# OllieBoyne/FIND

Hardware: AMD Instinct MI355X
Metric: deformed vertices x rendered views / sec (fwd+bwd) (higher is better)
Workload: dtype f32; 1 GPU; train_3d.yaml network-stage step: 16 feet x 6890-vertex template per GPU, 10002-vertex GT scans, chamf(5000)+smooth+texture(1000) losses, backward, Adam(main_params) step; nothing rendered, views:=1; feet_per_gpu=16, template_verts=6890, parallelism=dp1

## Files before the change

find_amd/csrc/geom.hip:

```cpp
#include "common.h"

namespace find {
namespace geom {

__device__ __forceinline__ float3 ld3(const float* p) { return make_float3(p[0], p[1], p[2]); }
__device__ __forceinline__ float3 sub3(float3 a, float3 b) { return make_float3(a.x - b.x, a.y - b.y, a.z - b.z); }
__device__ __forceinline__ float3 cross3(float3 a, float3 b) {
	return make_float3(a.y * b.z - a.z * b.y, a.z * b.x - a.x * b.z, a.x * b.y - a.y * b.x);
}
__device__ __forceinline__ float norm3(float3 a) { return sqrtf(a.x * a.x + a.y * a.y + a.z * a.z); }

__global__ void face_areas_kernel(const float* __restrict__ verts, const int32_t* __restrict__ faces, int64_t faces_mesh_stride,
								  int n_verts, int n_faces, float* __restrict__ areas) {
	const int m = blockIdx.y;
	const int f = blockIdx.x * blockDim.x + threadIdx.x;
	if (f >= n_faces) return;
	const int32_t* fp = faces + (int64_t)m * faces_mesh_stride + (int64_t)f * 3;
	const float* vp = verts + (int64_t)m * n_verts * 3;
	if (fp[0] < 0) {
		areas[(int64_t)m * n_faces + f] = 0.f;
		return;
	}
	const float3 a = ld3(vp + 3 * fp[0]), b = ld3(vp + 3 * fp[1]), c = ld3(vp + 3 * fp[2]);
	areas[(int64_t)m * n_faces + f] = 0.5f * norm3(cross3(sub3(b, a), sub3(c, a)));
// ... 419 lines not shown
					if (nn_dist(fx, fy, fz, s[0], s[1], s[2]) == best[k]) jj = j;
				}
			}
			key[k] = nn_key(best[k], jj);
		}
	}
	if (wave) {
#pragma unroll
		for (int k = 0; k < NQ; ++k) pkey[wave - 1][k * 64 + lane] = key[k];
	}
	__syncthreads();
	if (wave == 0) {
		float* dist = dir ? a.d[1].dist : a.d[0].dist;
		int32_t* idx = dir ? a.d[1].idx : a.d[0].idx;
		unsigned long long* kout = dir ? a.d[1].key : a.d[0].key;
#pragma unroll
		for (int k = 0; k < NQ; ++k) {
			unsigned long long b = key[k];
#pragma unroll
			for (int w = 0; w < 3; ++w) b = min(b, pkey[w][k * 64 + lane]);
			if (qi[k] >= p1_max) continue;
			const int64_t o = (int64_t)n * p1_max + qi[k];
			const bool valid = qi[k] < p1 && b != ~0ull;
			if (kout) {
				if (a.splits == 1) kout[o] = qi[k] < p1 ? b : ~0ull;
				else if (valid) atomicMin(kout + o, b);
			}
			if (dist) dist[o] = valid ? __uint_as_float((unsigned)(b >> 32)) : 0.f;
			if (idx) idx[o] = valid ? (int)(unsigned)b : -1;
		}
	}
}

__global__ __launch_bounds__(1024) void chamfer_reduce_kernel(const unsigned long long* __restrict__ kx, const int32_t* __restrict__ x_len, int p1_max,
															  const unsigned long long* __restrict__ ky, const int32_t* __restrict__ y_len, int p2_max,
															  int n_clouds, float* __restrict__ partial, unsigned* __restrict__ counter,
															  float* __restrict__ loss) {
	__shared__ float red[16];
	__shared__ bool last;
	const int n = blockIdx.x, dir = blockIdx.y;
	const unsigned long long* k = dir ? ky : kx;
	const int32_t* len = dir ? y_len : x_len;
	const int pmax = dir ? p2_max : p1_max;
	const int p = len ? len[n] : pmax;
	float s = 0.f;
	for (int i = threadIdx.x; i < p; i += 1024) {
		const unsigned long long v = k[(int64_t)n * pmax + i];
		s += v == ~0ull ? 0.f : __uint_as_float((unsigned)(v >> 32));
	}
	s = wave_sum(s);
	if ((threadIdx.x & 63) == 0) red[threadIdx.x >> 6] = s;
	__syncthreads();
	if (threadIdx.x == 0) {
		float t = 0.f;
		for (int w = 0; w < 16; ++w) t += red[w];
		partial[dir * n_clouds + n] = t / (float)max(p, 1);
		__threadfence();
		last = atomicAdd(counter, 1u) == 2u * n_clouds - 1u;
	}
	__syncthreads();
	if (last && threadIdx.x == 0) {
		__threadfence();
		float total = 0.f;
		for (int i = 0; i < 2 * n_clouds; ++i) total += __builtin_nontemporal_load(partial + i);
		*loss = total / (float)max(n_clouds, 1);
	}
// ... 212 lines not shown
__global__ __launch_bounds__(256) void chamfer_surface_sum_kernel(const float* __restrict__ slabs, int n_slices, int64_t slab_stride, int V3,
																  float* __restrict__ d_verts) {
	const int n = blockIdx.y, e = blockIdx.x * 256 + threadIdx.x;
	if (e >= V3) return;
	const float* p = slabs + (int64_t)n * n_slices * slab_stride + e;
	float s = 0.f;
	for (int k = 0; k < n_slices; ++k) s += p[(int64_t)k * slab_stride];
	d_verts[(int64_t)n * V3 + e] = s;
}

__global__ void nn_bwd_kernel(const float* __restrict__ x, const int32_t* __restrict__ x_len, const float* __restrict__ y,
							  const int32_t* __restrict__ idx, const float* __restrict__ w, int p1_max, int p2_max,
							  float* __restrict__ d_x, float* __restrict__ d_y) {
	const int n = blockIdx.y;
	const int i = blockIdx.x * blockDim.x + threadIdx.x;
	const int p1 = x_len ? x_len[n] : p1_max;
	if (i >= p1) return;
	const int64_t o = (int64_t)n * p1_max + i;
	const int j = idx[o];
	if (j < 0) return;
	const float g = 2.0f * w[o];
	const float* xp = x + o * 3;
	const float* yp = y + ((int64_t)n * p2_max + j) * 3;
	const float gx = g * (xp[0] - yp[0]), gy = g * (xp[1] - yp[1]), gz = g * (xp[2] - yp[2]);
	if (d_x) {
		d_x[o * 3 + 0] += gx; d_x[o * 3 + 1] += gy; d_x[o * 3 + 2] += gz;
	}
	if (d_y) {
		float* dy = d_y + ((int64_t)n * p2_max + j) * 3;
		atomicAdd(dy + 0, -gx); atomicAdd(dy + 1, -gy); atomicAdd(dy + 2, -gz);
	}
}

__global__ void cot_weights_kernel(const float* __restrict__ verts, const int32_t* __restrict__ faces, int n_verts, int n_faces,
								   float* __restrict__ fw) {
#pragma clang fp contract(off)
	const int m = blockIdx.y;
	const int f = blockIdx.x * blockDim.x + threadIdx.x;
	if (f >= n_faces) return;
	const int32_t* fp = faces + (int64_t)f * 3;
	const float* vp = verts + (int64_t)m * n_verts * 3;
	const float3 v0 = ld3(vp + 3 * fp[0]), v1 = ld3(vp + 3 * fp[1]), v2 = ld3(vp + 3 * fp[2]);
	const float A = norm3(sub3(v1, v2)), B = norm3(sub3(v0, v2)), C = norm3(sub3(v0, v1));
	const float s = 0.5f * (A + B + C);
	const float area = sqrtf(fmaxf(s * (s - A) * (s - B) * (s - C), 1e-12f));
	const float A2 = A * A, B2 = B * B, C2 = C * C;
	float* o = fw + ((int64_t)m * n_faces + f) * 3;
	o[0] = (B2 + C2 - A2) / area / 4.0f;
	o[1] = (A2 + C2 - B2) / area / 4.0f;
	o[2] = (A2 + B2 - C2) / area / 4.0f;
}

__device__ __forceinline__ float quad_sum(float v) {
	v += __shfl_xor(v, 1, 64);
	v += __shfl_xor(v, 2, 64);
	return v;
}

template <typename Q>
__device__ __forceinline__ void apply_L(Q qv, const int32_t* __restrict__ faces, const float* __restrict__ fw,
										const int32_t* __restrict__ vf_off, const int32_t* __restrict__ vf_items, int i, int t, bool live,
										float3* r, float* rowsum) {
	float3 acc = make_float3(0.f, 0.f, 0.f);
	float rs = 0.f;
	if (live) {
		const int hi = vf_off[i + 1];
		for (int e = vf_off[i] + t; e < hi; e += 4) {
			const int item = vf_items[e];
			const int f = item / 3, c = item - f * 3;
			const int c1 = (c + 1) % 3, c2 = (c + 2) % 3;
			const int j1 = faces[f * 3 + c1], j2 = faces[f * 3 + c2];
			const float w1 = fw[f * 3 + c2], w2 = fw[f * 3 + c1];
			const float3 a = qv(j1), b = qv(j2);
			acc.x += w1 * a.x + w2 * b.x; acc.y += w1 * a.y + w2 * b.y; acc.z += w1 * a.z + w2 * b.z;
			rs += w1 + w2;
		}
	}
	*r = make_float3(quad_sum(acc.x), quad_sum(acc.y), quad_sum(acc.z));
	*rowsum = quad_sum(rs);
}

constexpr int SMOOTH_VPB = 64;

__global__ __launch_bounds__(256) void smooth_fwd_kernel(const float* __restrict__ verts, const int32_t* __restrict__ faces,
														   const float* __restrict__ fw, const int32_t* __restrict__ vf_off,
														   const int32_t* __restrict__ vf_items, const int32_t* __restrict__ nbr_off,
														   const int32_t* __restrict__ nbr_idx, int n_verts, int n_faces,
														   float* __restrict__ nw_out, float* __restrict__ lapdir_out,
														   float* __restrict__ partial ) {
	const int m = blockIdx.y;
	const int i = blockIdx.x * SMOOTH_VPB + ((int)threadIdx.x >> 2), t = threadIdx.x & 3;
	const bool live = i < n_verts;
	const float* vp = verts + (int64_t)m * n_verts * 3;
	float3 r;
	float rs;
	apply_L([&](int j) { return ld3(vp + 3 * j); }, faces, fw + (int64_t)m * n_faces * 3, vf_off, vf_items, i, t, live, &r, &rs);
	float lap_n = 0.f, edge_s = 0.f;
	if (live) {
		const float3 v = ld3(vp + 3 * i);
		const int hi = nbr_off[i + 1];
		for (int e = nbr_off[i] + t; e < hi; e += 4) {
			const float3 d = sub3(v, ld3(vp + 3 * nbr_idx[e]));
			edge_s += d.x * d.x + d.y * d.y + d.z * d.z;
		}
		if (t == 0) {
			const float nw = rs > 0.f ? 1.0f / rs : rs;
			const float3 lap = make_float3(r.x * nw - v.x, r.y * nw - v.y, r.z * nw - v.z);
			lap_n = norm3(lap);
			const float inv = lap_n > 0.f ? 1.0f / lap_n : 0.f;
			const int64_t o = (int64_t)m * n_verts + i;
			nw_out[o] = nw;
			lapdir_out[o * 3 + 0] = lap.x * inv; lapdir_out[o * 3 + 1] = lap.y * inv; lapdir_out[o * 3 + 2] = lap.z * inv;
		}
	}
	__shared__ float red[2][4];
	const float a = wave_sum(lap_n), b = wave_sum(edge_s);
	if ((threadIdx.x & 63) == 0) { red[0][threadIdx.x >> 6] = a; red[1][threadIdx.x >> 6] = b; }
	__syncthreads();
	if (threadIdx.x < 2) {
		float sum = 0.f;
		for (int w = 0; w < 4; ++w) sum += red[threadIdx.x][w];
		partial[((int64_t)m * gridDim.x + blockIdx.x) * 2 + threadIdx.x] = sum;
	}
}

__global__ void smooth_finalize_kernel(const float* __restrict__ partial, int n_meshes, int nblk, int n_verts, int n_edges,
									   float* __restrict__ loss_edge, float* __restrict__ loss_lap, float w_edge, float w_lap,
									   float* __restrict__ loss_sum) {
	float lap = 0.f, edge = 0.f;
	for (int k = threadIdx.x; k < n_meshes * nblk; k += 64) { lap += partial[k * 2 + 0]; edge += partial[k * 2 + 1]; }
	lap = wave_sum(lap);
	edge = wave_sum(edge);
	if (threadIdx.x == 0) {
		const float l = lap / (float)n_verts / (float)n_meshes, e = 0.5f * edge / (float)n_edges / (float)n_meshes;
		if (loss_lap) *loss_lap = l;
		if (loss_edge) *loss_edge = e;
		if (loss_sum) *loss_sum = w_lap * l + w_edge * e;
	}
}

__global__ __launch_bounds__(256) void smooth_bwd_kernel(const float* __restrict__ verts, const int32_t* __restrict__ faces,
														   const float* __restrict__ fw, const int32_t* __restrict__ vf_off,
														   const int32_t* __restrict__ vf_items, const int32_t* __restrict__ nbr_off,
														   const int32_t* __restrict__ nbr_idx, const float* __restrict__ nw,
														   const float* __restrict__ lapdir, const float* __restrict__ g_edge,
														   const float* __restrict__ g_lap, float s_edge, float s_lap, int n_meshes, int n_verts,
														   int n_faces, int n_edges, float* __restrict__ d_verts) {
	const int m = blockIdx.y;
	const int i = blockIdx.x * SMOOTH_VPB + ((int)threadIdx.x >> 2), t = threadIdx.x & 3;
	const bool live = i < n_verts;
	const float* vp = verts + (int64_t)m * n_verts * 3;
	const float* nwp = nw + (int64_t)m * n_verts;
	const float* ldp = lapdir + (int64_t)m * n_verts * 3;
	const float su = (*g_lap) * s_lap / (float)n_verts / (float)n_meshes;
	float3 r;
	float rs;
	apply_L([&](int j) { const float sj = su * nwp[j]; const float3 u = ld3(ldp + 3 * j); return make_float3(sj * u.x, sj * u.y, sj * u.z); },
			faces, fw + (int64_t)m * n_faces * 3, vf_off, vf_items, i, t, live, &r, &rs);
	float3 es = make_float3(0.f, 0.f, 0.f);
	float3 v = es;
	if (live) {
		v = ld3(vp + 3 * i);
		const int hi = nbr_off[i + 1];
		for (int e = nbr_off[i] + t; e < hi; e += 4) {
			const float3 d = sub3(v, ld3(vp + 3 * nbr_idx[e]));
			es.x += d.x; es.y += d.y; es.z += d.z;
		}
	}
	es = make_float3(quad_sum(es.x), quad_sum(es.y), quad_sum(es.z));
	if (live && t == 0) {
		const int64_t o = (int64_t)m * n_verts + i;
		const float se = 2.0f * (*g_edge) * s_edge / (float)n_edges / (float)n_meshes;
		d_verts[o * 3 + 0] = r.x - su * ldp[3 * i + 0] + se * es.x;
		d_verts[o * 3 + 1] = r.y - su * ldp[3 * i + 1] + se * es.y;
		d_verts[o * 3 + 2] = r.z - su * ldp[3 * i + 2] + se * es.z;
	}
}

struct SmoothWs {
	float* fw;
	float* nw;
	float* lapdir;
	float* partial;
	int nblk;
	int64_t bytes;
};

static void carve_smooth(int64_t n_meshes, int64_t n_verts, int64_t n_faces, void* ws, SmoothWs* o) {
	Carver c(ws);
	o->nblk = (int)cdiv(n_verts, SMOOTH_VPB);
	o->fw = c.take<float>(n_meshes * n_faces * 3);
	o->nw = c.take<float>(n_meshes * n_verts);
	o->lapdir = c.take<float>(n_meshes * n_verts * 3);
	o->partial = c.take<float>(n_meshes * o->nblk * 2);
	o->bytes = c.off;
}

}
}

using namespace find;
using namespace find::geom;

static inline bool bad_dims(int64_t a, int64_t b) { return a < 1 || b < 1 || a >= (1 << 16) || b >= (1ll << 30); }

extern "C" int find_face_areas(const float* verts, const int32_t* faces, int64_t faces_batch, int64_t n_meshes, int64_t n_verts,
							   int64_t n_faces, float* areas, void* stream) {
	FIND_REQUIRE(verts && faces && areas, "find_face_areas: NULL argument");
	FIND_REQUIRE(!bad_dims(n_meshes, n_faces) && n_verts >= 1, "find_face_areas: bad sizes");
	FIND_REQUIRE(faces_batch == 1 || faces_batch == n_meshes, "find_face_areas: faces_batch must be 1 or n_meshes");
	hipLaunchKernelGGL(face_areas_kernel, dim3((unsigned)cdiv(n_faces, 256), (unsigned)n_meshes), dim3(256), 0, (hipStream_t)stream, verts,
					   faces, faces_batch == 1 ? 0 : n_faces * 3, (int)n_verts, (int)n_faces, areas);
	FIND_LAUNCH_CHECK("face_areas_kernel");
	return FIND_OK;
}

extern "C" int find_sample_points_fwd(const float* verts, const int32_t* faces, int64_t faces_batch, const int32_t* face_idx,
									  const float* uv, int64_t n_meshes, int64_t n_verts, int64_t n_faces, int64_t n_samples,
									  float* out, const float* attr, float* attr_out, void* stream) {
	FIND_REQUIRE(verts && faces && face_idx && uv && out, "find_sample_points_fwd: NULL argument");
	FIND_REQUIRE((attr == nullptr) == (attr_out == nullptr), "find_sample_points_fwd: attr and attr_out must both be given or both NULL");
	FIND_REQUIRE(!bad_dims(n_meshes, n_samples) && n_verts >= 1 && n_faces >= 1, "find_sample_points_fwd: bad sizes");
	FIND_REQUIRE(faces_batch == 1 || faces_batch == n_meshes, "find_sample_points_fwd: faces_batch must be 1 or n_meshes");
	hipLaunchKernelGGL(sample_fwd_kernel, dim3((unsigned)cdiv(n_samples, 256), (unsigned)n_meshes), dim3(256), 0, (hipStream_t)stream, verts,
					   faces, faces_batch == 1 ? 0 : n_faces * 3, face_idx, uv, (int)n_verts, (int)n_samples, out, attr, attr_out);
	FIND_LAUNCH_CHECK("sample_fwd_kernel");
	return FIND_OK;
// ... 146 lines not shown
				const bool face = (z == cz - r) || (z == cz + r) || (yy == cy - r) || (yy == cy + r);
				if (face || r == 0) scan_row(z, yy, x0, x1);
				else {
					if (cx - r >= 0) scan_row(z, yy, cx - r, cx - r);
					if (cx + r <= NG - 1) scan_row(z, yy, cx + r, cx + r);
				}
			}
		if (x0 == 0 && x1 == NG - 1 && y0 == 0 && y1 == NG - 1 && z0 == 0 && z1 == NG - 1) break;
		float gap = INFINITY;
		const float mx = 1e-4f * clx + 6e-7f * fmaxf(fabsf(ox), fabsf(qx)), my = 1e-4f * cly + 6e-7f * fmaxf(fabsf(oy), fabsf(qy)),
					mz = 1e-4f * clz + 6e-7f * fmaxf(fabsf(oz), fabsf(qz));
		if (cx - r > 0) gap = fminf(gap, rx - (cx - r) * clx - mx);
		if (cx + r < NG - 1) gap = fminf(gap, (cx + r + 1) * clx - rx - mx);
		if (cy - r > 0) gap = fminf(gap, ry - (cy - r) * cly - my);
		if (cy + r < NG - 1) gap = fminf(gap, (cy + r + 1) * cly - ry - my);
		if (cz - r > 0) gap = fminf(gap, rz - (cz - r) * clz - mz);
		if (cz + r < NG - 1) gap = fminf(gap, (cz + r + 1) * clz - rz - mz);
		gap = fmaxf(gap, 0.f);
		if (best != ~0ull && __uint_as_float((unsigned)(best >> 32)) < gap * gap * 0.9999f) break;
	}
	kout[qi] = best;
}

constexpr int TILE_PTS = 64;
constexpr int TILE_MAX_TILES = 128;
constexpr int TILE_MAX_POINTS = TILE_PTS * TILE_MAX_TILES;
struct TileDir {
	const float* p;
	const int32_t* len;
	int p_max;
	float4* sorted;
	float4* tab;
};
struct TileBuildArgs { TileDir d[2]; };

__device__ __forceinline__ unsigned tile_ord(float f) {
	const unsigned b = __float_as_uint(f);
	return b ^ ((b >> 31) ? 0xffffffffu : 0x80000000u);
}
__device__ __forceinline__ float tile_unord(unsigned u) { return __uint_as_float(u ^ ((u >> 31) ? 0x80000000u : 0xffffffffu)); }
__device__ __forceinline__ int tile_bin(float v, float lo, float scale) { return (int)fminf(fmaxf((v - lo) * scale, 0.f), 63.f); }

__device__ __forceinline__ unsigned tile_wave_max(unsigned v) {
	v = max(v, (unsigned)__builtin_amdgcn_update_dpp(0, (int)v, 0xB1, 0xf, 0xf, true));
	v = max(v, (unsigned)__builtin_amdgcn_update_dpp(0, (int)v, 0x4E, 0xf, 0xf, true));
	v = max(v, (unsigned)__builtin_amdgcn_update_dpp(0, (int)v, 0x141, 0xf, 0xf, true));
	v = max(v, (unsigned)__builtin_amdgcn_update_dpp(0, (int)v, 0x140, 0xf, 0xf, true));
	return max(max((unsigned)__builtin_amdgcn_readlane((int)v, 0), (unsigned)__builtin_amdgcn_readlane((int)v, 16)),
			   max((unsigned)__builtin_amdgcn_readlane((int)v, 32), (unsigned)__builtin_amdgcn_readlane((int)v, 48)));
}

__device__ __forceinline__ int tile_wave_scan(int v, int lane) {
	v += __builtin_amdgcn_update_dpp(0, v, 0x111, 0xf, 0xf, true);
	v += __builtin_amdgcn_update_dpp(0, v, 0x112, 0xf, 0xf, true);
	v += __builtin_amdgcn_update_dpp(0, v, 0x114, 0xf, 0xf, true);
	v += __builtin_amdgcn_update_dpp(0, v, 0x118, 0xf, 0xf, true);
	const int r0 = __builtin_amdgcn_readlane(v, 15), r1 = __builtin_amdgcn_readlane(v, 31), r2 = __builtin_amdgcn_readlane(v, 47);
	return v + (lane >= 16 ? r0 : 0) + (lane >= 32 ? r1 : 0) + (lane >= 48 ? r2 : 0);
}
__device__ __forceinline__ int tile_widest(float ex, float ey, float ez) {
	return (ey > ex && ey >= ez) ? 1 : (ez > ex && ez > ey) ? 2 : 0;
}

__global__ __launch_bounds__(1024) void nn_tile_build_kernel(const TileBuildArgs a) {
	constexpr int PPT = TILE_MAX_POINTS / 1024, MT = TILE_MAX_TILES;
	__shared__ int hist[MT / 2 * 64];
	__shared__ int n_m[2][MT];
	__shared__ int n_cnt[MT], n_start[MT], n_axis[MT];
	__shared__ float n_lo[3][MT], n_hi[3][MT];
	__shared__ float4 n_par[MT];
	__shared__ int4 s_split[MT];
	__shared__ int s_taken[MT];
	__shared__ unsigned b_lo[3][MT], b_hi[3][MT];
	__shared__ unsigned red[6][16];
	const int dir = blockIdx.y, n = blockIdx.x;
	const float* __restrict__ pts = dir ? a.d[1].p : a.d[0].p;
	const int32_t* len = dir ? a.d[1].len : a.d[0].len;
	const int p_max = dir ? a.d[1].p_max : a.d[0].p_max;
	const int p = min(max(len ? len[n] : p_max, 0), p_max);
	const int M = (p + TILE_PTS - 1) / TILE_PTS;
	if (M == 0 || M > MT) return;
	float4* sorted = (dir ? a.d[1].sorted : a.d[0].sorted) + (int64_t)n * p_max;
	float4* tab = (dir ? a.d[1].tab : a.d[0].tab) + (int64_t)n * ((p_max + TILE_PTS - 1) / TILE_PTS) * 2;
	const float* pp = pts + (int64_t)n * p_max * 3;
	const int tid = threadIdx.x, lane = tid & 63, wave = tid >> 6;
	const int kmax = (p + 1023) >> 10;
	float px[PPT], py[PPT], pz[PPT];
	int node[PPT], bin[PPT];
	bool own[PPT];
	float lo[3] = {INFINITY, INFINITY, INFINITY}, hi[3] = {-INFINITY, -INFINITY, -INFINITY};
#pragma unroll
	for (int k = 0; k < PPT; ++k) {
		const int j = k * 1024 + tid;
		own[k] = j < p;
		node[k] = 0;
		bin[k] = 0;
		const int jj = min(j, p - 1);
		px[k] = pp[(int64_t)jj * 3]; py[k] = pp[(int64_t)jj * 3 + 1]; pz[k] = pp[(int64_t)jj * 3 + 2];
		lo[0] = fminf(lo[0], px[k]); hi[0] = fmaxf(hi[0], px[k]);
		lo[1] = fminf(lo[1], py[k]); hi[1] = fmaxf(hi[1], py[k]);
		lo[2] = fminf(lo[2], pz[k]); hi[2] = fmaxf(hi[2], pz[k]);
	}
#pragma unroll
	for (int c = 0; c < 3; ++c) {
		const unsigned l = tile_wave_max(~tile_ord(lo[c])), h = tile_wave_max(tile_ord(hi[c]));
		if (lane == 0) { red[c][wave] = l; red[3 + c][wave] = h; }
	}
	for (int i = tid; i < MT / 2 * 64; i += 1024) hist[i] = 0;
	if (tid < MT) {
		n_m[0][tid] = 0; n_m[1][tid] = 0; s_taken[tid] = 0;
		s_split[tid] = make_int4(0, 0, 0, 0);
#pragma unroll
		for (int c = 0; c < 3; ++c) { b_lo[c][tid] = 0xffffffffu; b_hi[c][tid] = 0u; }
// ... 97 lines not shown
	__syncthreads();
	int pos[PPT];
#pragma unroll
	for (int k = 0; k < PPT; ++k) pos[k] = own[k] ? n_start[node[k]] + atomicAdd(&s_taken[node[k]], 1) : -1;
#pragma unroll
	for (int k = 0; k < PPT; ++k) {
		if (!own[k]) continue;
		const int f = node[k];
		atomicMin(&b_lo[0][f], tile_ord(px[k])); atomicMax(&b_hi[0][f], tile_ord(px[k]));
		atomicMin(&b_lo[1][f], tile_ord(py[k])); atomicMax(&b_hi[1][f], tile_ord(py[k]));
		atomicMin(&b_lo[2][f], tile_ord(pz[k])); atomicMax(&b_hi[2][f], tile_ord(pz[k]));
	}
#pragma unroll
	for (int k = 0; k < PPT; ++k)
		if (pos[k] >= 0 && pos[k] < p) sorted[pos[k]] = make_float4(px[k], py[k], pz[k], __int_as_float(k * 1024 + tid));
	__syncthreads();
	if (tid < M) {
		tab[2 * tid] = make_float4(tile_unord(b_lo[0][tid]), tile_unord(b_lo[1][tid]), tile_unord(b_lo[2][tid]), __int_as_float(n_start[tid]));
		tab[2 * tid + 1] = make_float4(tile_unord(b_hi[0][tid]), tile_unord(b_hi[1][tid]), tile_unord(b_hi[2][tid]), __int_as_float(n_cnt[tid]));
	}
}

struct TileQueryDir {
	const float4* qsorted;
	const float4* qtab;
	const int32_t* q_len;
	int q_max;
	const float4* tsorted;
	const float4* ttab;
	const int32_t* t_len;
	int t_max;
	unsigned long long* key;
};
struct TileQueryArgs { TileQueryDir d[2]; unsigned* counter; };

__global__ __launch_bounds__(256) void nn_tile_query_kernel(const TileQueryArgs a) {
	__shared__ float4 tl[4][TILE_PTS / 8 * 6];
	__shared__ int ti[4][TILE_PTS];
	const int dir = blockIdx.z, n = blockIdx.y;
	if (a.counter && (blockIdx.x | blockIdx.y | blockIdx.z | threadIdx.x) == 0) *a.counter = 0u;
	const int q_max = dir ? a.d[1].q_max : a.d[0].q_max, t_max = dir ? a.d[1].t_max : a.d[0].t_max;
	const int32_t* q_len = dir ? a.d[1].q_len : a.d[0].q_len;
	const int32_t* t_len = dir ? a.d[1].t_len : a.d[0].t_len;
	const int p1 = min(max(q_len ? q_len[n] : q_max, 0), q_max), p2 = min(max(t_len ? t_len[n] : t_max, 0), t_max);
	unsigned long long* kout = (dir ? a.d[1].key : a.d[0].key) + (int64_t)n * q_max;
	for (int r = p1 + blockIdx.x * 256 + threadIdx.x; r < q_max; r += gridDim.x * 256) kout[r] = ~0ull;
	const int lane = threadIdx.x & 63, wave = threadIdx.x >> 6;
	const int qt = __builtin_amdgcn_readfirstlane(blockIdx.x * 4 + wave);
	if (qt >= (p1 + TILE_PTS - 1) / TILE_PTS) return;
	const float4* __restrict__ qsorted = (dir ? a.d[1].qsorted : a.d[0].qsorted) + (int64_t)n * q_max;
	const float4* __restrict__ qtab = (dir ? a.d[1].qtab : a.d[0].qtab) + (int64_t)n * ((q_max + TILE_PTS - 1) / TILE_PTS) * 2;
	const float4* __restrict__ tsorted = (dir ? a.d[1].tsorted : a.d[0].tsorted) + (int64_t)n * t_max;
	const float4* __restrict__ ttab = (dir ? a.d[1].ttab : a.d[0].ttab) + (int64_t)n * ((t_max + TILE_PTS - 1) / TILE_PTS) * 2;
	const float4 qb0 = qtab[2 * qt], qb1 = qtab[2 * qt + 1];
	const int qstart = __builtin_amdgcn_readfirstlane(__float_as_int(qb0.w)), qcnt = __builtin_amdgcn_readfirstlane(__float_as_int(qb1.w));
	if (qcnt <= 0) return;
	const float4 q = qsorted[min(max(qstart, 0) + min(lane, qcnt - 1), p1 - 1)];
	const int ntt = (p2 + TILE_PTS - 1) / TILE_PTS;
	float lb[2];
	int tstart[2], tcnt[2];
#pragma unroll
	for (int h = 0; h < 2; ++h) {
		const int t = h * 64 + lane;
		lb[h] = INFINITY; tstart[h] = 0; tcnt[h] = 0;
		if (t < ntt) {
			const float4 b0 = ttab[2 * t], b1 = ttab[2 * t + 1];
			const float gx = fmaxf(0.f, fmaxf(b0.x - qb1.x, qb0.x - b1.x)), gy = fmaxf(0.f, fmaxf(b0.y - qb1.y, qb0.y - b1.y)),
						gz = fmaxf(0.f, fmaxf(b0.z - qb1.z, qb0.z - b1.z));
			lb[h] = __builtin_fmaf(gz, gz, __builtin_fmaf(gy, gy, gx * gx));
			tstart[h] = __float_as_int(b0.w); tcnt[h] = __float_as_int(b1.w);
		}
	}
	unsigned ord[2] = {lane < ntt ? __float_as_uint(lb[0]) : ~0u, 64 + lane < ntt ? __float_as_uint(lb[1]) : ~0u};
	unsigned picked_lb = ~0u;
	auto pick = [&]() -> int {
		picked_lb = ~tile_wave_max(~min(ord[0], ord[1]));
		if (picked_lb == ~0u) return -1;
		const unsigned long long b0 = __ballot(ord[0] == picked_lb);
		const int tt = b0 ? __builtin_ctzll(b0) : 64 + __builtin_ctzll(__ballot(ord[1] == picked_lb));
		if (lane == (tt & 63)) { if (tt < 64) ord[0] = ~0u; else ord[1] = ~0u; }
		return tt;
	};
	const v2f qx = {q.x, q.x}, qy = {q.y, q.y}, qz = {q.z, q.z};
	float best = INFINITY;
	int gj = 0;
	unsigned long long tie = ~0ull;
	float4* L = tl[wave];
	int* LI = ti[wave];
	float4 v = make_float4(0.f, 0.f, 0.f, 0.f);
// ... 29 lines not shown
			const int gn = min(g + 1, ng - 1);
#pragma unroll
			for (int i = 0; i < 6; ++i) B[i] = L[6 * gn + i];
#define FIND_TILE_D2(X, Y, Z, lo, hi) ({ const v2f dx = qx - v2f{X.lo, X.hi}, dy = qy - v2f{Y.lo, Y.hi}, dz = qz - v2f{Z.lo, Z.hi};   \
										 __builtin_elementwise_fma(dz, dz, __builtin_elementwise_fma(dy, dy, dx * dx)); })
			const v2f d0 = FIND_TILE_D2(A[0], A[2], A[4], x, y), d1 = FIND_TILE_D2(A[0], A[2], A[4], z, w);
			const v2f d2 = FIND_TILE_D2(A[1], A[3], A[5], x, y), d3 = FIND_TILE_D2(A[1], A[3], A[5], z, w);
#undef FIND_TILE_D2
			const float m = fminf(fminf(fminf(d0.x, d0.y), fminf(d1.x, d1.y)), fminf(fminf(d2.x, d2.y), fminf(d3.x, d3.y)));
			if (m == best) {
				const float dd[8] = {d0.x, d0.y, d1.x, d1.y, d2.x, d2.y, d3.x, d3.y};
#pragma unroll
				for (int c = 0; c < 8; ++c)
					if (dd[c] == best) tie = min(tie, nn_key(dd[c], LI[8 * g + c]));
			}
			if (m < best) { best = m; gj = base + 8 * g; }
#pragma unroll
			for (int i = 0; i < 6; ++i) A[i] = B[i];
		}
		if (t >= 0 && t_lb > tile_wave_max(__float_as_uint(best))) t = -1;
	}
	unsigned long long key = tie;
	if (ntt > 0) {
#pragma unroll
		for (int c = 0; c < 8; ++c) {
			const int j = gj + c;
			if (j < p2) {
				const float4 s = tsorted[j];
				key = min(key, nn_key(nn_dist(q.x, q.y, q.z, s.x, s.y, s.z), __float_as_int(s.w)));
			}
		}
	}
	const int qi = __float_as_int(q.w);
	if (lane < qcnt && qi >= 0 && qi < p1) kout[qi] = key;
}

static void nn_shape(int64_t blocks_np1, int64_t p2_max, int* np, int* splits) {
	*np = blocks_np1 >= 4096 ? 2 : 1;
	*splits = 1;
	while (blocks_np1 * *splits < 512 && *splits < 8 && p2_max / (*splits * 2) >= 256) *splits *= 2;
}

static int launch_nn(const NnArgs& a, int np, int64_t p_max, int64_t n, hipStream_t s) {
	const dim3 grid((unsigned)cdiv(p_max, 128 * np), (unsigned)n, (unsigned)(a.n_dirs * a.splits));
	if (np == 2) hipLaunchKernelGGL(nn_kernel<2>, grid, dim3(256), 0, s, a);
	else hipLaunchKernelGGL(nn_kernel<1>, grid, dim3(256), 0, s, a);
	return check_launch("nn_kernel");
}

extern "C" int find_nn_fwd(const float* x, const int32_t* x_len, const float* y, const int32_t* y_len, int64_t n, int64_t p1_max,
						   int64_t p2_max, float* dist, int32_t* idx, void* stream) {
	FIND_REQUIRE(x && y && dist && idx, "find_nn_fwd: NULL argument");
	FIND_REQUIRE(!bad_dims(n, p1_max) && p2_max >= 1 && p2_max < (1ll << 30), "find_nn_fwd: bad sizes");
	NnArgs a = {};
	a.d[0] = NnDir{x, x_len, y, y_len, (int)p1_max, (int)p2_max, dist, idx, nullptr};
	a.n_dirs = 1;
	int np, splits;
	nn_shape(cdiv(p1_max, 128) * n, p2_max, &np, &splits);
	a.splits = 1;
	return launch_nn(a, np, p1_max, n, (hipStream_t)stream);
}

extern "C" int find_nn_bwd(const float* x, const int32_t* x_len, const float* y, const int32_t* idx, const float* w, int64_t n,
						   int64_t p1_max, int64_t p2_max, float* d_x, float* d_y, void* stream) {
	FIND_REQUIRE(x && y && idx && w, "find_nn_bwd: NULL argument");
	FIND_REQUIRE(d_x || d_y, "find_nn_bwd: both gradient outputs NULL");
	FIND_REQUIRE(!bad_dims(n, p1_max) && p2_max >= 1, "find_nn_bwd: bad sizes");
	hipLaunchKernelGGL(nn_bwd_kernel, dim3((unsigned)cdiv(p1_max, 256), (unsigned)n), dim3(256), 0, (hipStream_t)stream, x, x_len, y, idx, w,
					   (int)p1_max, (int)p2_max, d_x, d_y);
	FIND_LAUNCH_CHECK("nn_bwd_kernel");
	return FIND_OK;
}

struct ChamferWs {
	unsigned long long* kx;
	unsigned long long* ky;
	int64_t key_bytes;
	float* partial;
	unsigned* counter;
	float4 *sorted_x, *sorted_y;
	int32_t *cells_x, *cells_y;
	float *box_x, *box_y;
	float4 *tab_x, *tab_y;
	int64_t bytes;
};
constexpr int64_t GRID_MIN_POINTS = 8192;
constexpr int64_t TILE_MIN_POINTS = 2048, TILE_MIN_PAIRS = 300000000;
static bool tile_path(int64_t n, int64_t p1_max, int64_t p2_max) {
	if (g_raster_ablate & (512 | 32768)) return false;
	if (std::max(p1_max, p2_max) > TILE_MAX_POINTS) return false;
	if (g_raster_ablate & 16384) return std::min(p1_max, p2_max) >= 64;
	if (g_raster_ablate & 1024) return false;
	return n * p1_max * p2_max >= TILE_MIN_PAIRS && std::min(p1_max, p2_max) >= TILE_MIN_POINTS && std::max(p1_max, p2_max) < GRID_MIN_POINTS;
}
static void carve_chamfer(int64_t n, int64_t p1_max, int64_t p2_max, void* ws, ChamferWs* o) {
	Carver c(ws);
	o->kx = c.take<unsigned long long>(n * p1_max);
	o->ky = c.take<unsigned long long>(n * p2_max);
	o->key_bytes = c.off;
	o->partial = c.take<float>(2 * n);
	o->counter = c.take<unsigned>(1);
	o->sorted_x = c.take<float4>(n * p1_max);
	o->sorted_y = c.take<float4>(n * p2_max);
	o->cells_x = c.take<int32_t>(n * (NG3 + 1));
	o->cells_y = c.take<int32_t>(n * (NG3 + 1));
	o->box_x = c.take<float>(n * 8);
	o->box_y = c.take<float>(n * 8);
	o->tab_x = c.take<float4>(n * cdiv(p1_max, TILE_PTS) * 2);
	o->tab_y = c.take<float4>(n * cdiv(p2_max, TILE_PTS) * 2);
	o->bytes = c.off;
}

extern "C" int64_t find_chamfer_ws_bytes(int64_t n, int64_t p1_max, int64_t p2_max) {
	if (bad_dims(n, p1_max) || bad_dims(n, p2_max)) return -1;
	ChamferWs w;
	carve_chamfer(n, p1_max, p2_max, nullptr, &w);
	return w.bytes;
}

extern "C" int find_chamfer_fwd(const float* x, const int32_t* x_len, const float* y, const int32_t* y_len, int64_t n, int64_t p1_max, int64_t p2_max,
								float* loss, void* ws, int64_t ws_bytes, void* stream) {
	FIND_REQUIRE(x && y && loss && ws, "find_chamfer_fwd: NULL argument");
	FIND_REQUIRE(!bad_dims(n, p1_max) && !bad_dims(n, p2_max), "find_chamfer_fwd: bad sizes");
	ChamferWs w;
	carve_chamfer(n, p1_max, p2_max, ws, &w);
	if (ws_bytes < w.bytes) { set_error("find_chamfer_fwd: workspace too small"); return FIND_EWORKSPACE; }
	hipStream_t s = (hipStream_t)stream;
	if (tile_path(n, p1_max, p2_max)) {
		TileBuildArgs b = {};
		b.d[0] = TileDir{x, x_len, (int)p1_max, w.sorted_x, w.tab_x};
		b.d[1] = TileDir{y, y_len, (int)p2_max, w.sorted_y, w.tab_y};
		hipLaunchKernelGGL(nn_tile_build_kernel, dim3((unsigned)n, 2), dim3(1024), 0, s, b);
		FIND_LAUNCH_CHECK("nn_tile_build_kernel");
		TileQueryArgs q = {};
		q.d[0] = TileQueryDir{w.sorted_x, w.tab_x, x_len, (int)p1_max, w.sorted_y, w.tab_y, y_len, (int)p2_max, w.kx};
		q.d[1] = TileQueryDir{w.sorted_y, w.tab_y, y_len, (int)p2_max, w.sorted_x, w.tab_x, x_len, (int)p1_max, w.ky};
		q.counter = w.counter;
		hipLaunchKernelGGL(nn_tile_query_kernel, dim3((unsigned)cdiv(cdiv(std::max(p1_max, p2_max), TILE_PTS), 4), (unsigned)n, 2), dim3(256), 0, s, q);
		FIND_LAUNCH_CHECK("nn_tile_query_kernel");
		hipLaunchKernelGGL(chamfer_reduce_kernel, dim3((unsigned)n, 2), dim3(1024), 0, s, w.kx, x_len, (int)p1_max, w.ky, y_len, (int)p2_max, (int)n, w.partial, w.counter,
						   loss);
		FIND_LAUNCH_CHECK("chamfer_reduce_kernel");
		return FIND_OK;
	}
	const int64_t grid_from = (g_raster_ablate & 1024) ? 64 : GRID_MIN_POINTS;
	if (p1_max >= grid_from && p2_max >= grid_from && !(g_raster_ablate & 512)) {
		GridBuildArgs b = {};
		b.d[0] = GridDir{y, y_len, (int)p2_max, w.sorted_y, w.cells_y, w.box_y};
		b.d[1] = GridDir{x, x_len, (int)p1_max, w.sorted_x, w.cells_x, w.box_x};
		hipLaunchKernelGGL(nn_grid_build_kernel, dim3((unsigned)n, 2), dim3(1024), 0, s, b);
		FIND_LAUNCH_CHECK("nn_grid_build_kernel");
		GridQueryArgs q = {};
		q.d[0] = GridQueryDir{x, x_len, (int)p1_max, (int)p2_max, w.sorted_y, w.cells_y, w.box_y, w.kx};
		q.d[1] = GridQueryDir{y, y_len, (int)p2_max, (int)p1_max, w.sorted_x, w.cells_x, w.box_x, w.ky};
		q.counter = w.counter;
		hipLaunchKernelGGL(nn_grid_query_kernel, dim3((unsigned)cdiv(std::max(p1_max, p2_max), 256), (unsigned)n, 2), dim3(256), 0, s, q);
		FIND_LAUNCH_CHECK("nn_grid_query_kernel");
		hipLaunchKernelGGL(chamfer_reduce_kernel, dim3((unsigned)n, 2), dim3(1024), 0, s, w.kx, x_len, (int)p1_max, w.ky, y_len, (int)p2_max, (int)n, w.partial, w.counter,
						   loss);
		FIND_LAUNCH_CHECK("chamfer_reduce_kernel");
		return FIND_OK;
	}
	NnArgs a = {};
	a.d[0] = NnDir{x, x_len, y, y_len, (int)p1_max, (int)p2_max, nullptr, nullptr, w.kx};
	a.d[1] = NnDir{y, y_len, x, x_len, (int)p2_max, (int)p1_max, nullptr, nullptr, w.ky};
	a.n_dirs = 2;
	a.counter = w.counter;
	const int64_t p_max = std::max(p1_max, p2_max);
	int np;
	nn_shape(cdiv(p_max, 128) * n * 2, std::min(p1_max, p2_max), &np, &a.splits);
	if (a.splits > 1) {
		hipError_t e = hipMemsetAsync(ws, 0xff, (size_t)w.key_bytes, s);
		if (e != hipSuccess) { set_error("find_chamfer_fwd: hipMemsetAsync: %s", hipGetErrorString(e)); return FIND_ELAUNCH; }
	}
	int rc = launch_nn(a, np, p_max, n, s);
// ... 152 lines not shown
								  const float* g_loss, float* d_a, float* d_a_mask, void* stream) {
	FIND_REQUIRE(a && b && g_loss && (d_a || d_a_mask), "find_image_mse_bwd: NULL argument");
	FIND_REQUIRE(n_pix >= 1 && n_pix < (1ll << 40) && channels >= 1 && channels <= 16, "find_image_mse_bwd: bad sizes");
	FIND_REQUIRE(!d_a_mask || a_mask, "find_image_mse_bwd: d_a_mask without a_mask");
	hipStream_t s = (hipStream_t)stream;
	const bool vec = (n_pix & 3) == 0 && (channels == 3 || channels == 1) && al16(a) && al16(b) && al16(a_mask) && al16(b_mask) && al16(d_a) && al16(d_a_mask);
	if (vec && channels == 3)
		hipLaunchKernelGGL((image_mse_bwd_kernel<3, true>), dim3((unsigned)cdiv(n_pix >> 2, 256)), dim3(256), 0, s, a, a_mask, b, b_mask, n_pix, 3, g_loss, d_a, d_a_mask);
	else if (vec)
		hipLaunchKernelGGL((image_mse_bwd_kernel<1, true>), dim3((unsigned)cdiv(n_pix >> 2, 256)), dim3(256), 0, s, a, a_mask, b, b_mask, n_pix, 1, g_loss, d_a, d_a_mask);
	else
		hipLaunchKernelGGL((image_mse_bwd_kernel<1, false>), dim3((unsigned)cdiv(n_pix, 256)), dim3(256), 0, s, a, a_mask, b, b_mask, n_pix, (int)channels, g_loss, d_a,
						   d_a_mask);
	FIND_LAUNCH_CHECK("image_mse_bwd_kernel");
	return FIND_OK;
}

extern "C" int64_t find_smooth_ws_bytes(int64_t n_meshes, int64_t n_verts, int64_t n_faces) {
	if (bad_dims(n_meshes, n_verts) || n_faces < 1) return -1;
	SmoothWs w;
	carve_smooth(n_meshes, n_verts, n_faces, nullptr, &w);
	return w.bytes;
}

static int smooth_fwd_body(const char* who, const float* verts, const int32_t* faces, const int32_t* vf_off, const int32_t* vf_items, const int32_t* nbr_off,
						   const int32_t* nbr_idx, int64_t n_meshes, int64_t n_verts, int64_t n_faces, int64_t n_edges, float* loss_edge, float* loss_lap,
						   float w_edge, float w_lap, float* loss_sum, void* ws, int64_t ws_bytes, void* stream) {
	FIND_REQUIRE(verts && faces && vf_off && vf_items && nbr_off && nbr_idx && ws, "%s: NULL argument", who);
	FIND_REQUIRE(!bad_dims(n_meshes, n_verts) && n_faces >= 1 && n_edges >= 1, "%s: bad sizes", who);
	SmoothWs w;
	carve_smooth(n_meshes, n_verts, n_faces, ws, &w);
	if (ws_bytes < w.bytes) { set_error("%s: workspace too small", who); return FIND_EWORKSPACE; }
	hipStream_t s = (hipStream_t)stream;
	hipLaunchKernelGGL(cot_weights_kernel, dim3((unsigned)cdiv(n_faces, 256), (unsigned)n_meshes), dim3(256), 0, s, verts, faces, (int)n_verts, (int)n_faces, w.fw);
	hipLaunchKernelGGL(smooth_fwd_kernel, dim3((unsigned)w.nblk, (unsigned)n_meshes), dim3(256), 0, s, verts, faces, w.fw, vf_off, vf_items, nbr_off,
					   nbr_idx, (int)n_verts, (int)n_faces, w.nw, w.lapdir, w.partial);
	hipLaunchKernelGGL(smooth_finalize_kernel, dim3(1), dim3(64), 0, s, w.partial, (int)n_meshes, w.nblk, (int)n_verts, (int)n_edges, loss_edge, loss_lap,
					   w_edge, w_lap, loss_sum);
	FIND_LAUNCH_CHECK(who);
	return FIND_OK;
}

static int smooth_bwd_body(const char* who, const float* verts, const int32_t* faces, const int32_t* vf_off, const int32_t* vf_items, const int32_t* nbr_off,
						   const int32_t* nbr_idx, int64_t n_meshes, int64_t n_verts, int64_t n_faces, int64_t n_edges, const float* g_edge, const float* g_lap,
						   float s_edge, float s_lap, void* ws, int64_t ws_bytes, float* d_verts, void* stream) {
	FIND_REQUIRE(verts && faces && vf_off && vf_items && nbr_off && nbr_idx && g_edge && g_lap && ws && d_verts, "%s: NULL argument", who);
	FIND_REQUIRE(!bad_dims(n_meshes, n_verts) && n_faces >= 1 && n_edges >= 1, "%s: bad sizes", who);
	SmoothWs w;
	carve_smooth(n_meshes, n_verts, n_faces, ws, &w);
	if (ws_bytes < w.bytes) { set_error("%s: workspace too small", who); return FIND_EWORKSPACE; }
	hipStream_t s = (hipStream_t)stream;
	hipLaunchKernelGGL(smooth_bwd_kernel, dim3((unsigned)cdiv(n_verts, SMOOTH_VPB), (unsigned)n_meshes), dim3(256), 0, s, verts, faces, w.fw, vf_off, vf_items, nbr_off, nbr_idx,
					   w.nw, w.lapdir, g_edge, g_lap, s_edge, s_lap, (int)n_meshes, (int)n_verts, (int)n_faces, (int)n_edges, d_verts);
	FIND_LAUNCH_CHECK(who);
	return FIND_OK;
}

extern "C" int find_smooth_fwd(const float* verts, const int32_t* faces, const int32_t* vf_off, const int32_t* vf_items,
							   const int32_t* nbr_off, const int32_t* nbr_idx, int64_t n_meshes, int64_t n_verts, int64_t n_faces,
							   int64_t n_edges, float* loss_edge, float* loss_lap, void* ws, int64_t ws_bytes, void* stream) {
	FIND_REQUIRE(loss_edge && loss_lap, "find_smooth_fwd: NULL argument");
	return smooth_fwd_body("find_smooth_fwd", verts, faces, vf_off, vf_items, nbr_off, nbr_idx, n_meshes, n_verts, n_faces, n_edges, loss_edge, loss_lap, 0.f, 0.f,
						   nullptr, ws, ws_bytes, stream);
}

extern "C" int find_smooth_bwd(const float* verts, const int32_t* faces, const int32_t* vf_off, const int32_t* vf_items,
							   const int32_t* nbr_off, const int32_t* nbr_idx, int64_t n_meshes, int64_t n_verts, int64_t n_faces,
							   int64_t n_edges, const float* g_edge, const float* g_lap, void* ws, int64_t ws_bytes, float* d_verts,
							   void* stream) {
	return smooth_bwd_body("find_smooth_bwd", verts, faces, vf_off, vf_items, nbr_off, nbr_idx, n_meshes, n_verts, n_faces, n_edges, g_edge, g_lap, 1.f, 1.f, ws,
						   ws_bytes, d_verts, stream);
// ... 17 lines not shown
```

Measured before the change: 75.70 million vertices*views/s.

## Fuse chamfer and smooth loss reductions into producer kernels via last-block counters

Removes the separate chamfer_reduce and smooth_finalize launches by having the last-arriving block of the tile query and smooth forward kernels perform the final reduction. Agent-scope atomic counters (reset by the preceding build/cot kernels) and relaxed atomic stores with acquire fences order the partial results. This cuts two kernel launches per step and the inter-kernel gaps, in exchange for extra synchronisation logic, a serial tail in the last block, and ordering-correctness risk.

```diff
diff --git a/find_amd/csrc/geom.hip b/find_amd/csrc/geom.hip
--- a/find_amd/csrc/geom.hip
+++ b/find_amd/csrc/geom.hip
@@ -475,6 +475,34 @@
 	}
 }
 
+__device__ __forceinline__ void st_agent(float* p, float v) {
+	__hip_atomic_store(reinterpret_cast<unsigned*>(p), __float_as_uint(v), __ATOMIC_RELAXED, __HIP_MEMORY_SCOPE_AGENT);
+}
+__device__ __forceinline__ void st_agent(unsigned long long* p, unsigned long long v) { __hip_atomic_store(p, v, __ATOMIC_RELAXED, __HIP_MEMORY_SCOPE_AGENT); }
+__device__ __forceinline__ float ld_agent(const float* p) {
+	return __uint_as_float(__hip_atomic_load(reinterpret_cast<const unsigned*>(p), __ATOMIC_RELAXED, __HIP_MEMORY_SCOPE_AGENT));
+}
+__device__ __forceinline__ bool arrive_lane(unsigned* counter, unsigned expected) {
+	const bool last = __hip_atomic_fetch_add(counter, 1u, __ATOMIC_RELAXED, __HIP_MEMORY_SCOPE_AGENT) == expected - 1u;
+	if (last) __hip_atomic_store(counter, 0u, __ATOMIC_RELAXED, __HIP_MEMORY_SCOPE_AGENT);
+	return last;
+}
+__device__ __forceinline__ void acquire_lane() {
+	__builtin_amdgcn_fence(__ATOMIC_ACQUIRE, "agent");
+	asm volatile("s_waitcnt vmcnt(0)" ::: "memory");
+}
+__device__ __forceinline__ bool arrive_last(unsigned* counter, unsigned expected, unsigned* flag) {
+	asm volatile("s_waitcnt vmcnt(0)" ::: "memory");
+	__syncthreads();
+	if (threadIdx.x == 0) {
+		const bool last = arrive_lane(counter, expected);
+		if (last) acquire_lane();
+		*flag = last ? 1u : 0u;
+	}
+	__syncthreads();
+	return *flag != 0u;
+}
+
 __global__ __launch_bounds__(1024) void chamfer_reduce_kernel(const unsigned long long* __restrict__ kx, const int32_t* __restrict__ x_len, int p1_max,
 															  const unsigned long long* __restrict__ ky, const int32_t* __restrict__ y_len, int p2_max,
 															  int n_clouds, float* __restrict__ partial, unsigned* __restrict__ counter,
@@ -753,11 +781,14 @@
 	}
 }
 
+constexpr int SMOOTH_COUNTER_STRIDE = 64;
 __global__ void cot_weights_kernel(const float* __restrict__ verts, const int32_t* __restrict__ faces, int n_verts, int n_faces,
-								   float* __restrict__ fw) {
+								   float* __restrict__ fw, unsigned* __restrict__ counter) {
 #pragma clang fp contract(off)
 	const int m = blockIdx.y;
 	const int f = blockIdx.x * blockDim.x + threadIdx.x;
+	if ((blockIdx.x | blockIdx.y) == 0)
+		for (int i = threadIdx.x; i < 1 + (int)gridDim.y; i += blockDim.x) counter[i * SMOOTH_COUNTER_STRIDE] = 0u;
 	if (f >= n_faces) return;
 	const int32_t* fp = faces + (int64_t)f * 3;
 	const float* vp = verts + (int64_t)m * n_verts * 3;
@@ -803,12 +834,36 @@
 
 constexpr int SMOOTH_VPB = 64;
 
+__device__ __forceinline__ void smooth_finalize(const float* partial, int n_meshes, int nblk, int n_verts, int n_edges, float* loss_edge,
+												float* loss_lap, float w_edge, float w_lap, float* loss_sum) {
+	float lap = 0.f, edge = 0.f;
+	const int n = n_meshes * nblk;
+	for (int k0 = threadIdx.x; k0 < n; k0 += 64 * 8) {
+		float2 v[8];
+#pragma unroll
+		for (int u = 0; u < 8; ++u) v[u] = reinterpret_cast<const float2*>(partial)[min(k0 + 64 * u, n - 1)];
+#pragma unroll
+		for (int u = 0; u < 8; ++u)
+			if (k0 + 64 * u < n) { lap += v[u].x; edge += v[u].y; }
+	}
+	lap = wave_sum(lap);
+	edge = wave_sum(edge);
+	if (threadIdx.x == 0) {
+		const float l = lap / (float)n_verts / (float)n_meshes, e = 0.5f * edge / (float)n_edges / (float)n_meshes;
+		if (loss_lap) *loss_lap = l;
+		if (loss_edge) *loss_edge = e;
+		if (loss_sum) *loss_sum = w_lap * l + w_edge * e;
+	}
+}
+
 __global__ __launch_bounds__(256) void smooth_fwd_kernel(const float* __restrict__ verts, const int32_t* __restrict__ faces,
 														   const float* __restrict__ fw, const int32_t* __restrict__ vf_off,
 														   const int32_t* __restrict__ vf_items, const int32_t* __restrict__ nbr_off,
 														   const int32_t* __restrict__ nbr_idx, int n_verts, int n_faces,
 														   float* __restrict__ nw_out, float* __restrict__ lapdir_out,
-														   float* __restrict__ partial ) {
+														   float* partial , unsigned* counter, int n_edges,
+														   float* __restrict__ loss_edge, float* __restrict__ loss_lap, float w_edge, float w_lap,
+														   float* __restrict__ loss_sum) {
 	const int m = blockIdx.y;
 	const int i = blockIdx.x * SMOOTH_VPB + ((int)threadIdx.x >> 2), t = threadIdx.x & 3;
 	const bool live = i < n_verts;
@@ -841,23 +896,17 @@
 	if (threadIdx.x < 2) {
 		float sum = 0.f;
 		for (int w = 0; w < 4; ++w) sum += red[threadIdx.x][w];
-		partial[((int64_t)m * gridDim.x + blockIdx.x) * 2 + threadIdx.x] = sum;
-	}
-}
-
-__global__ void smooth_finalize_kernel(const float* __restrict__ partial, int n_meshes, int nblk, int n_verts, int n_edges,
-									   float* __restrict__ loss_edge, float* __restrict__ loss_lap, float w_edge, float w_lap,
-									   float* __restrict__ loss_sum) {
-	float lap = 0.f, edge = 0.f;
-	for (int k = threadIdx.x; k < n_meshes * nblk; k += 64) { lap += partial[k * 2 + 0]; edge += partial[k * 2 + 1]; }
-	lap = wave_sum(lap);
-	edge = wave_sum(edge);
-	if (threadIdx.x == 0) {
-		const float l = lap / (float)n_verts / (float)n_meshes, e = 0.5f * edge / (float)n_edges / (float)n_meshes;
-		if (loss_lap) *loss_lap = l;
-		if (loss_edge) *loss_edge = e;
-		if (loss_sum) *loss_sum = w_lap * l + w_edge * e;
-	}
+		st_agent(partial + ((int64_t)m * gridDim.x + blockIdx.x) * 2 + threadIdx.x, sum);
+	}
+	if (threadIdx.x >= 64) return;
+	asm volatile("s_waitcnt vmcnt(0)" ::: "memory");
+	int last = 0;
+	if (threadIdx.x == 0 && arrive_lane(counter + (1 + m) * SMOOTH_COUNTER_STRIDE, gridDim.x) && arrive_lane(counter, gridDim.y)) {
+		acquire_lane();
+		last = 1;
+	}
+	if (!__builtin_amdgcn_readfirstlane(last)) return;
+	smooth_finalize(partial, (int)gridDim.y, (int)gridDim.x, n_verts, n_edges, loss_edge, loss_lap, w_edge, w_lap, loss_sum);
 }
 
 __global__ __launch_bounds__(256) void smooth_bwd_kernel(const float* __restrict__ verts, const int32_t* __restrict__ faces,
@@ -903,6 +952,7 @@
 	float* nw;
 	float* lapdir;
 	float* partial;
+	unsigned* counter;
 	int nblk;
 	int64_t bytes;
 };
@@ -914,6 +964,7 @@
 	o->nw = c.take<float>(n_meshes * n_verts);
 	o->lapdir = c.take<float>(n_meshes * n_verts * 3);
 	o->partial = c.take<float>(n_meshes * o->nblk * 2);
+	o->counter = c.take<unsigned>((1 + n_meshes) * SMOOTH_COUNTER_STRIDE);
 	o->bytes = c.off;
 }
 
@@ -1126,7 +1177,7 @@
 	float4* sorted;
 	float4* tab;
 };
-struct TileBuildArgs { TileDir d[2]; };
+struct TileBuildArgs { TileDir d[2]; unsigned* counter;  };
 
 __device__ __forceinline__ unsigned tile_ord(float f) {
 	const unsigned b = __float_as_uint(f);
@@ -1173,6 +1224,8 @@
 	const int p_max = dir ? a.d[1].p_max : a.d[0].p_max;
 	const int p = min(max(len ? len[n] : p_max, 0), p_max);
 	const int M = (p + TILE_PTS - 1) / TILE_PTS;
+	if ((blockIdx.x | blockIdx.y) == 0)
+		for (int i = threadIdx.x; i < 1 + 2 * (int)gridDim.x; i += 1024) a.counter[i] = 0u;
 	if (M == 0 || M > MT) return;
 	float4* sorted = (dir ? a.d[1].sorted : a.d[0].sorted) + (int64_t)n * p_max;
 	float4* tab = (dir ? a.d[1].tab : a.d[0].tab) + (int64_t)n * ((p_max + TILE_PTS - 1) / TILE_PTS) * 2;
@@ -1336,29 +1389,31 @@
 	int t_max;
 	unsigned long long* key;
 };
-struct TileQueryArgs { TileQueryDir d[2]; unsigned* counter; };
+struct TileQueryArgs { TileQueryDir d[2]; unsigned* counter;  float* partial; float* loss; };
 
 __global__ __launch_bounds__(256) void nn_tile_query_kernel(const TileQueryArgs a) {
 	__shared__ float4 tl[4][TILE_PTS / 8 * 6];
 	__shared__ int ti[4][TILE_PTS];
-	const int dir = blockIdx.z, n = blockIdx.y;
-	if (a.counter && (blockIdx.x | blockIdx.y | blockIdx.z | threadIdx.x) == 0) *a.counter = 0u;
+	__shared__ float red[16];
+	__shared__ unsigned last;
+	const int dir = blockIdx.z, n = blockIdx.y, n_clouds = (int)gridDim.y;
 	const int q_max = dir ? a.d[1].q_max : a.d[0].q_max, t_max = dir ? a.d[1].t_max : a.d[0].t_max;
 	const int32_t* q_len = dir ? a.d[1].q_len : a.d[0].q_len;
 	const int32_t* t_len = dir ? a.d[1].t_len : a.d[0].t_len;
 	const int p1 = min(max(q_len ? q_len[n] : q_max, 0), q_max), p2 = min(max(t_len ? t_len[n] : t_max, 0), t_max);
 	unsigned long long* kout = (dir ? a.d[1].key : a.d[0].key) + (int64_t)n * q_max;
-	for (int r = p1 + blockIdx.x * 256 + threadIdx.x; r < q_max; r += gridDim.x * 256) kout[r] = ~0ull;
+	for (int r = p1 + blockIdx.x * 256 + threadIdx.x; r < q_max; r += gridDim.x * 256) st_agent(kout + r, ~0ull);
 	const int lane = threadIdx.x & 63, wave = threadIdx.x >> 6;
+	do {
 	const int qt = __builtin_amdgcn_readfirstlane(blockIdx.x * 4 + wave);
-	if (qt >= (p1 + TILE_PTS - 1) / TILE_PTS) return;
+	if (qt >= (p1 + TILE_PTS - 1) / TILE_PTS) break;
 	const float4* __restrict__ qsorted = (dir ? a.d[1].qsorted : a.d[0].qsorted) + (int64_t)n * q_max;
 	const float4* __restrict__ qtab = (dir ? a.d[1].qtab : a.d[0].qtab) + (int64_t)n * ((q_max + TILE_PTS - 1) / TILE_PTS) * 2;
 	const float4* __restrict__ tsorted = (dir ? a.d[1].tsorted : a.d[0].tsorted) + (int64_t)n * t_max;
 	const float4* __restrict__ ttab = (dir ? a.d[1].ttab : a.d[0].ttab) + (int64_t)n * ((t_max + TILE_PTS - 1) / TILE_PTS) * 2;
 	const float4 qb0 = qtab[2 * qt], qb1 = qtab[2 * qt + 1];
 	const int qstart = __builtin_amdgcn_readfirstlane(__float_as_int(qb0.w)), qcnt = __builtin_amdgcn_readfirstlane(__float_as_int(qb1.w));
-	if (qcnt <= 0) return;
+	if (qcnt <= 0) break;
 	const float4 q = qsorted[min(max(qstart, 0) + min(lane, qcnt - 1), p1 - 1)];
 	const int ntt = (p2 + TILE_PTS - 1) / TILE_PTS;
 	float lb[2];
@@ -1454,7 +1509,39 @@
 		}
 	}
 	const int qi = __float_as_int(q.w);
-	if (lane < qcnt && qi >= 0 && qi < p1) kout[qi] = key;
+	if (lane < qcnt && qi >= 0 && qi < p1) st_agent(kout + qi, key);
+	} while (false);
+
+	if (!arrive_last(a.counter + 1 + dir * n_clouds + n, gridDim.x, &last)) return;
+	const int p = q_len ? q_len[n] : q_max;
+	const int pe = min(p, q_max);
+#pragma unroll
+	for (int j = 0; j < 4; ++j) {
+		constexpr int PPT = TILE_MAX_POINTS / 1024;
+		unsigned long long v[PPT];
+#pragma unroll
+		for (int u = 0; u < PPT; ++u) {
+			const int i = j * 256 + (int)threadIdx.x + u * 1024;
+			v[u] = i < pe ? kout[i] : ~0ull;
+		}
+		float s = 0.f;
+#pragma unroll
+		for (int u = 0; u < PPT; ++u)
+			if (j * 256 + (int)threadIdx.x + u * 1024 < pe) s += v[u] == ~0ull ? 0.f : __uint_as_float((unsigned)(v[u] >> 32));
+		s = wave_sum(s);
+		if (lane == 0) red[4 * j + wave] = s;
+	}
+	__syncthreads();
+	if (threadIdx.x != 0) return;
+	float t = 0.f;
+	for (int w = 0; w < 16; ++w) t += red[w];
+	st_agent(a.partial + dir * n_clouds + n, t / (float)max(p, 1));
+	asm volatile("s_waitcnt vmcnt(0)" ::: "memory");
+	if (!arrive_lane(a.counter, 2u * n_clouds)) return;
+	acquire_lane();
+	float total = 0.f;
+	for (int i = 0; i < 2 * n_clouds; ++i) total += ld_agent(a.partial + i);
+	*a.loss = total / (float)max(n_clouds, 1);
 }
 
 static void nn_shape(int64_t blocks_np1, int64_t p2_max, int* np, int* splits) {
@@ -1521,7 +1608,7 @@
 	o->ky = c.take<unsigned long long>(n * p2_max);
 	o->key_bytes = c.off;
 	o->partial = c.take<float>(2 * n);
-	o->counter = c.take<unsigned>(1);
+	o->counter = c.take<unsigned>(1 + 2 * n);
 	o->sorted_x = c.take<float4>(n * p1_max);
 	o->sorted_y = c.take<float4>(n * p2_max);
 	o->cells_x = c.take<int32_t>(n * (NG3 + 1));
@@ -1552,17 +1639,15 @@
 		TileBuildArgs b = {};
 		b.d[0] = TileDir{x, x_len, (int)p1_max, w.sorted_x, w.tab_x};
 		b.d[1] = TileDir{y, y_len, (int)p2_max, w.sorted_y, w.tab_y};
+		b.counter = w.counter;
 		hipLaunchKernelGGL(nn_tile_build_kernel, dim3((unsigned)n, 2), dim3(1024), 0, s, b);
 		FIND_LAUNCH_CHECK("nn_tile_build_kernel");
 		TileQueryArgs q = {};
 		q.d[0] = TileQueryDir{w.sorted_x, w.tab_x, x_len, (int)p1_max, w.sorted_y, w.tab_y, y_len, (int)p2_max, w.kx};
 		q.d[1] = TileQueryDir{w.sorted_y, w.tab_y, y_len, (int)p2_max, w.sorted_x, w.tab_x, x_len, (int)p1_max, w.ky};
-		q.counter = w.counter;
+		q.counter = w.counter; q.partial = w.partial; q.loss = loss;
 		hipLaunchKernelGGL(nn_tile_query_kernel, dim3((unsigned)cdiv(cdiv(std::max(p1_max, p2_max), TILE_PTS), 4), (unsigned)n, 2), dim3(256), 0, s, q);
 		FIND_LAUNCH_CHECK("nn_tile_query_kernel");
-		hipLaunchKernelGGL(chamfer_reduce_kernel, dim3((unsigned)n, 2), dim3(1024), 0, s, w.kx, x_len, (int)p1_max, w.ky, y_len, (int)p2_max, (int)n, w.partial, w.counter,
-						   loss);
-		FIND_LAUNCH_CHECK("chamfer_reduce_kernel");
 		return FIND_OK;
 	}
 	const int64_t grid_from = (g_raster_ablate & 1024) ? 64 : GRID_MIN_POINTS;
@@ -1781,11 +1866,10 @@
 	carve_smooth(n_meshes, n_verts, n_faces, ws, &w);
 	if (ws_bytes < w.bytes) { set_error("%s: workspace too small", who); return FIND_EWORKSPACE; }
 	hipStream_t s = (hipStream_t)stream;
-	hipLaunchKernelGGL(cot_weights_kernel, dim3((unsigned)cdiv(n_faces, 256), (unsigned)n_meshes), dim3(256), 0, s, verts, faces, (int)n_verts, (int)n_faces, w.fw);
+	hipLaunchKernelGGL(cot_weights_kernel, dim3((unsigned)cdiv(n_faces, 256), (unsigned)n_meshes), dim3(256), 0, s, verts, faces, (int)n_verts, (int)n_faces, w.fw,
+					   w.counter);
 	hipLaunchKernelGGL(smooth_fwd_kernel, dim3((unsigned)w.nblk, (unsigned)n_meshes), dim3(256), 0, s, verts, faces, w.fw, vf_off, vf_items, nbr_off,
-					   nbr_idx, (int)n_verts, (int)n_faces, w.nw, w.lapdir, w.partial);
-	hipLaunchKernelGGL(smooth_finalize_kernel, dim3(1), dim3(64), 0, s, w.partial, (int)n_meshes, w.nblk, (int)n_verts, (int)n_edges, loss_edge, loss_lap,
-					   w_edge, w_lap, loss_sum);
+					   nbr_idx, (int)n_verts, (int)n_faces, w.nw, w.lapdir, w.partial, w.counter, (int)n_edges, loss_edge, loss_lap, w_edge, w_lap, loss_sum);
 	FIND_LAUNCH_CHECK(who);
 	return FIND_OK;
 }
```

Measured after the change: 75.55 million vertices*views/s. No clear change (-0.2%).
